# starkware-libs/stark-perpetual

Hardware: AMD Instinct MI355X
Metric: pedersen_hashes_per_sec (higher is better)
Workload: dtype u32x9; 1 GPU; 2^16-leaf Pedersen Merkle rebuild per GPU (BASELINE.json configs[1]), 63 rebuilds in lockstep; tree_height=16, leaves_per_gpu=65536, calls_per_region=28, streams=2, window_bits=26, combine=none

## Files before the change

### stark-perpetual_amd/csrc/curve.hpp

```cpp
#pragma once
#include "fp29.hpp"

namespace sp {

struct aff {
  fe x, y;
};
struct xyzz {
  fe X, Y, ZZ, ZZZ;
};
struct jac {
  fe X, Y, Z;
};

SP_HD xyzz xyzz_from_aff(const aff& p) {
  xyzz r;
  r.X = p.x;
  r.Y = p.y;
  r.ZZ = FE_ONE_M;
  r.ZZZ = FE_ONE_M;
  return r;
}

template <bool SCAN = false>
SP_HD xyzz xyzz_madd(const xyzz& a, const aff& q) {
  if constexpr (SCAN && SP_FE_SCAN) {
    fe t[3];
    fe_scan(t, scan_mul{q.x, a.ZZ}, scan_mul{q.y, a.ZZZ});
    const fe P = fe_sub(t[0], a.X), R = fe_sub(t[1], a.Y);
    const fe P2 = fe_dbl(P), R2 = fe_dbl(R);
    fe_scan(t, scan_sqr{P, P2}, scan_sqr{R, R2});
    const fe PP = t[0], RR = t[1];
    fe_scan(t, scan_mul{P, PP}, scan_mul{a.X, PP});
    const fe PPP = t[0], Q = t[1];
    xyzz r;
    r.X = fe_carry(fe_sub(fe_sub(RR, PPP), fe_dbl(Q)));
    const fe D = fe_sub(Q, r.X), nY = fe_neg_pinned(a.Y);
    fe_scan(t, scan_mul2{R, D, nY, PPP}, scan_mul{a.ZZ, PP}, scan_mul{a.ZZZ, PPP});
    r.Y = t[0];
    r.ZZ = t[1];
    r.ZZZ = t[2];
    return r;
  }
  const fe U2 = fe_mul_t<SCAN>(q.x, a.ZZ);
  const fe S2 = fe_mul_t<SCAN>(q.y, a.ZZZ);
  const fe P = fe_sub(U2, a.X);
  const fe R = fe_sub(S2, a.Y);
  const fe PP = fe_sqr_t<SCAN>(P);
  const fe PPP = fe_mul_t<SCAN>(P, PP);
  const fe Q = fe_mul_t<SCAN>(a.X, PP);
  xyzz r;
  r.X = fe_carry(fe_sub(fe_sub(fe_sqr_t<SCAN>(R), PPP), fe_dbl(Q)));
  r.Y = fe_mul_sub_mul_t<SCAN>(R, fe_sub(Q, r.X), a.Y, PPP);
  r.ZZ = fe_mul_t<SCAN>(a.ZZ, PP);
  r.ZZZ = fe_mul_t<SCAN>(a.ZZZ, PPP);
  return r;
}

template <bool SCAN = false>
SP_HD void xyzz_madd_x_only(const xyzz& a, const aff& q, fe& X3, fe& ZZ3) {
  if constexpr (SCAN && SP_FE_SCAN) {
    fe t[3];
    fe_scan(t, scan_mul{q.x, a.ZZ}, scan_mul{q.y, a.ZZZ});
    const fe P = fe_sub(t[0], a.X), R = fe_sub(t[1], a.Y);
    const fe P2 = fe_dbl(P), R2 = fe_dbl(R);
    fe_scan(t, scan_sqr{P, P2}, scan_sqr{R, R2});
    const fe PP = t[0], RR = t[1];
    fe_scan(t, scan_mul{P, PP}, scan_mul{a.X, PP}, scan_mul{a.ZZ, PP});
    X3 = fe_carry(fe_sub(fe_sub(RR, t[0]), fe_dbl(t[1])));
    ZZ3 = t[2];
    return;
  }
  const fe U2 = fe_mul_t<SCAN>(q.x, a.ZZ);
  const fe S2 = fe_mul_t<SCAN>(q.y, a.ZZZ);
  const fe P = fe_sub(U2, a.X);
  const fe R = fe_sub(S2, a.Y);
  const fe PP = fe_sqr_t<SCAN>(P);
  const fe PPP = fe_mul_t<SCAN>(P, PP);
  const fe Q = fe_mul_t<SCAN>(a.X, PP);
  X3 = fe_carry(fe_sub(fe_sub(fe_sqr_t<SCAN>(R), PPP), fe_dbl(Q)));
  ZZ3 = fe_mul_t<SCAN>(a.ZZ, PP);
}

template <bool SCAN = false>
SP_HD xyzz xyzz_mmadd(const aff& a, const aff& b) {
  if constexpr (SCAN && SP_FE_SCAN) {
    const fe P = fe_sub(b.x, a.x), R = fe_carry(fe_sub(b.y, a.y));
    const fe P2 = fe_dbl(P), R2 = fe_dbl(R);
    fe t[2];
    fe_scan(t, scan_sqr{P, P2}, scan_sqr{R, R2});
    const fe PP = t[0], RR = t[1];
    fe_scan(t, scan_mul{P, PP}, scan_mul{a.x, PP});
    const fe PPP = t[0], Q = t[1];
    xyzz r;
    r.X = fe_carry(fe_sub(fe_sub(RR, PPP), fe_dbl(Q)));
    r.Y = fe_mul_sub_mul_scan(R, fe_sub(Q, r.X), a.y, PPP);
    r.ZZ = PP;
    r.ZZZ = PPP;
    return r;
  }
  const fe P = fe_sub(b.x, a.x);
  const fe R = fe_carry(fe_sub(b.y, a.y));
  const fe PP = fe_sqr_t<SCAN>(P);
  const fe PPP = fe_mul_t<SCAN>(P, PP);
  const fe Q = fe_mul_t<SCAN>(a.x, PP);
  xyzz r;
  r.X = fe_carry(fe_sub(fe_sub(fe_sqr_t<SCAN>(R), PPP), fe_dbl(Q)));
  r.Y = fe_mul_sub_mul_t<SCAN>(R, fe_sub(Q, r.X), a.y, PPP);
  r.ZZ = PP;
  r.ZZZ = PPP;
  return r;
}

template <bool SCAN = false>
SP_HD xyzz xyzz_add(const xyzz& a, const xyzz& b) {
  const fe U1 = fe_mul_t<SCAN>(a.X, b.ZZ);
  const fe U2 = fe_mul_t<SCAN>(b.X, a.ZZ);
  const fe S1 = fe_mul_t<SCAN>(a.Y, b.ZZZ);
  const fe S2 = fe_mul_t<SCAN>(b.Y, a.ZZZ);
  const fe P = fe_sub(U2, U1);
  const fe R = fe_sub(S2, S1);
  const fe PP = fe_sqr_t<SCAN>(P);
  const fe PPP = fe_mul_t<SCAN>(P, PP);
  const fe Q = fe_mul_t<SCAN>(U1, PP);
  xyzz r;
  r.X = fe_carry(fe_sub(fe_sub(fe_sqr_t<SCAN>(R), PPP), fe_dbl(Q)));
  r.Y = fe_mul_sub_mul_t<SCAN>(R, fe_sub(Q, r.X), S1, PPP);
  r.ZZ = fe_mul_t<SCAN>(fe_mul_t<SCAN>(a.ZZ, b.ZZ), PP);
  r.ZZZ = fe_mul_t<SCAN>(fe_mul_t<SCAN>(a.ZZZ, b.ZZZ), PPP);
  return r;
}

template <bool SCAN = false>
SP_HD void xyzz_add_x_only(const xyzz& a, const xyzz& b, fe& X3, fe& ZZ3) {
  const fe U1 = fe_mul_t<SCAN>(a.X, b.ZZ);
  const fe U2 = fe_mul_t<SCAN>(b.X, a.ZZ);
  const fe S1 = fe_mul_t<SCAN>(a.Y, b.ZZZ);
  const fe S2 = fe_mul_t<SCAN>(b.Y, a.ZZZ);
  const fe P = fe_sub(U2, U1);
  const fe R = fe_sub(S2, S1);
  const fe PP = fe_sqr_t<SCAN>(P);
  const fe PPP = fe_mul_t<SCAN>(P, PP);
  const fe Q = fe_mul_t<SCAN>(U1, PP);
  X3 = fe_carry(fe_sub(fe_sub(fe_sqr_t<SCAN>(R), PPP), fe_dbl(Q)));
  ZZ3 = fe_mul_t<SCAN>(fe_mul_t<SCAN>(a.ZZ, b.ZZ), PP);
}

SP_HD jac jac_dbl(const jac& p, const fe& a_coef) {
  const fe XX = fe_sqr(p.X);
  const fe YY = fe_sqr(p.Y);
  const fe YYYY = fe_sqr(YY);
  const fe ZZ = fe_sqr(p.Z);
  const fe t0 = fe_carry(fe_add(p.X, YY));
  const fe halfS = fe_carry(fe_sub(fe_sub(fe_sqr(t0), XX), YYYY));
  const fe S = fe_carry(fe_dbl(halfS));
  const fe XX3 = fe_carry(fe_add(fe_dbl(XX), XX));
  const fe M = fe_carry(fe_add(XX3, fe_mul(a_coef, fe_sqr(ZZ))));
  jac r;
  r.X = fe_carry(fe_sub(fe_sqr(M), fe_dbl(S)));
  const fe y4 = fe_carry(fe_dbl(fe_dbl(YYYY)));
  r.Y = fe_carry(fe_sub(fe_mul(M, fe_sub(S, r.X)), fe_dbl(y4)));
  const fe t1 = fe_carry(fe_add(p.Y, p.Z));
  r.Z = fe_carry(fe_sub(fe_sub(fe_sqr(t1), YY), ZZ));
  return r;
}

struct mjac {
  fe X, Y, Z, W;
};
SP_HD mjac mjac_from(const jac& p, const fe& a_coef) {
  mjac m;
  m.X = p.X; m.Y = p.Y; m.Z = p.Z;
  m.W = fe_mul(a_coef, fe_sqr(fe_sqr(p.Z)));
  return m;
}
SP_HD void mjac_dbl(mjac& p, bool need_w) {
  const fe XX = fe_sqr(p.X);
  const fe YY = fe_sqr(p.Y);
  const fe YYYY = fe_sqr(YY);
  const fe S = fe_carry(fe_dbl(fe_carry(fe_dbl(fe_mul(p.X, YY)))));
  const fe U = fe_carry(fe_dbl(fe_carry(fe_dbl(fe_carry(fe_dbl(YYYY))))));
  const fe M = fe_carry(fe_add(fe_carry(fe_add(fe_dbl(XX), XX)), p.W));
  const fe X3 = fe_carry(fe_sub(fe_sqr(M), fe_dbl(S)));
  const fe Y3 = fe_carry(fe_sub(fe_mul(M, fe_carry(fe_sub(S, X3))), U));
  const fe Z3 = fe_carry(fe_dbl(fe_mul(p.Y, p.Z)));
  if (need_w) p.W = fe_carry(fe_dbl(fe_mul(U, p.W)));
  p.X = X3;
  p.Y = Y3;
  p.Z = Z3;
}

SP_HD jac jac_madd(const jac& p, const aff& q) {
  const fe Z1Z1 = fe_sqr(p.Z);
  const fe U2 = fe_mul(q.x, Z1Z1);
  const fe S2 = fe_mul(fe_mul(q.y, p.Z), Z1Z1);
  const fe H = fe_sub(U2, p.X);
  const fe HH = fe_sqr(H);
  const fe I = fe_dbl(fe_carry(fe_dbl(HH)));
  const fe J = fe_mul(H, I);
  const fe rr = fe_carry(fe_dbl(fe_sub(S2, p.Y)));
  const fe V = fe_mul(p.X, I);
  jac r;
  r.X = fe_carry(fe_sub(fe_sub(fe_sqr(rr), J), fe_dbl(V)));
  r.Y = fe_mul_sub_mul(rr, fe_sub(V, r.X), fe_carry(fe_dbl(p.Y)), J);
  const fe t = fe_carry(fe_add(p.Z, H));
  r.Z = fe_carry(fe_sub(fe_sub(fe_sqr(t), Z1Z1), HH));
  return r;
}

SP_HD jac jac_add(const jac& p, const jac& q) {
  const fe Z1Z1 = fe_sqr(p.Z);
  const fe Z2Z2 = fe_sqr(q.Z);
  const fe U1 = fe_mul(p.X, Z2Z2);
  const fe U2 = fe_mul(q.X, Z1Z1);
  const fe S1 = fe_mul(fe_mul(p.Y, q.Z), Z2Z2);
  const fe S2 = fe_mul(fe_mul(q.Y, p.Z), Z1Z1);
  const fe H = fe_sub(U2, U1);
  const fe I = fe_dbl(fe_carry(fe_dbl(fe_sqr(H))));
  const fe J = fe_mul(H, I);
  const fe rr = fe_carry(fe_dbl(fe_sub(S2, S1)));
  const fe V = fe_mul(U1, I);
  jac r;
  r.X = fe_carry(fe_sub(fe_sub(fe_sqr(rr), J), fe_dbl(V)));
  r.Y = fe_mul_sub_mul(rr, fe_sub(V, r.X), fe_carry(fe_dbl(S1)), J);
  const fe t = fe_carry(fe_add(p.Z, q.Z));
  r.Z = fe_mul(fe_carry(fe_sub(fe_sub(fe_sqr(t), Z1Z1), Z2Z2)), H);
  return r;
}

}
```

### stark-perpetual_amd/csrc/fp29.hpp

```cpp
#pragma once
#include <stdint.h>
#include <utility>

#if defined(__HIPCC__)
#include <hip/hip_runtime.h>
#define SP_HD __host__ __device__ __forceinline__
#else
#define SP_HD inline
#endif

#if defined(SP_CHECK_BOUNDS) && !defined(__HIPCC__)
#include <stdio.h>
#include <stdlib.h>
#define SP_CHK32(expr64)                                                        \
  do {                                                                          \
    long long v__ = (long long)(expr64);                                        \
    if (v__ > 2147483647LL || v__ < -2147483648LL) {                            \
      fprintf(stderr, "limb overflow at %s:%d\n", __FILE__, __LINE__);          \
      abort();                                                                  \
    }                                                                           \
  } while (0)
#define SP_CHK64(expr128)                                                       \
  do {                                                                          \
    __int128 v__ = (expr128);                                                   \
// ... 87 lines not shown
#pragma unroll
  for (int i = 0; i < NL; ++i) r.l[i] = -a.l[i];
  return r;
}
SP_HD fe fe_dbl(const fe& a) {
  fe r;
#pragma unroll
  for (int i = 0; i < NL; ++i) { SP_CHK32((int64_t)a.l[i] * 2); r.l[i] = a.l[i] * 2; }
  return r;
}

SP_HD fe fe_carry(const fe& a) {
  fe r;
  int32_t c = 0;
#pragma unroll
  for (int i = 0; i < 8; ++i) {
    SP_CHK32((int64_t)a.l[i] + c);
    int32_t v = a.l[i] + c;
    r.l[i] = (int32_t)((uint32_t)v & LMASK);
    c = v >> LB;
  }
  r.l[8] = a.l[8] + c;
  return r;
}

SP_HD fe fe_weak_reduce(const fe& a) {
  const int32_t q = a.l[8] >> 19;
  fe r = a;
  r.l[0] -= q;
  r.l[6] -= q * P6;
  r.l[8] -= q * P8;
  return fe_carry(r);
}

SP_HD fe fe_half(const fe& a_in) {
  fe a = fe_carry(a_in);
  const int32_t odd = a.l[0] & 1;
  a.l[0] += odd;
  a.l[6] += odd * P6;
  a.l[8] += odd * P8;
  a = fe_carry(a);
  fe r;
#pragma unroll
  for (int i = 0; i < 8; ++i) r.l[i] = (int32_t)(((uint32_t)a.l[i] >> 1) | (((uint32_t)a.l[i + 1] & 1u) << (LB - 1)));
  r.l[8] = a.l[8] >> 1;
  return r;
}

struct cols {
  int64_t c[17];
};

SP_HD void cols_zero(cols& t) {
#pragma unroll
  for (int i = 0; i < 17; ++i) t.c[i] = 0;
}
SP_HD void cols_mac(cols& t, const fe& a, const fe& b) {
#pragma unroll
  for (int i = 0; i < NL; ++i)
#pragma unroll
    for (int j = 0; j < NL; ++j) {
      SP_CHK64((__int128)t.c[i + j] + (__int128)a.l[i] * b.l[j]);
      t.c[i + j] += (int64_t)a.l[i] * (int64_t)b.l[j];
    }
}
SP_HD void cols_msub(cols& t, const fe& a, const fe& b) {
#pragma unroll
  for (int i = 0; i < NL; ++i)
#pragma unroll
    for (int j = 0; j < NL; ++j) {
      SP_CHK64((__int128)t.c[i + j] - (__int128)a.l[i] * b.l[j]);
      t.c[i + j] -= (int64_t)a.l[i] * (int64_t)b.l[j];
    }
}
SP_HD void cols_sqr(cols& t, const fe& a) {
#pragma unroll
  for (int i = 0; i < NL; ++i) {
    SP_CHK64((__int128)t.c[2 * i] + (__int128)a.l[i] * a.l[i]);
    t.c[2 * i] += (int64_t)a.l[i] * (int64_t)a.l[i];
    SP_CHK32((int64_t)a.l[i] * 2);
    const int32_t d = a.l[i] * 2;
#pragma unroll
    for (int j = i + 1; j < NL; ++j) {
      SP_CHK64((__int128)t.c[i + j] + (__int128)d * a.l[j]);
      t.c[i + j] += (int64_t)d * (int64_t)a.l[j];
    }
  }
}

SP_HD fe fe_reduce(cols& t) {
  int32_t np6 = -P6, np8 = -P8;
#if defined(__HIP_DEVICE_COMPILE__)
  asm volatile("" : "+s"(np6), "+s"(np8));
#endif
#pragma unroll
  for (int i = 0; i < NL; ++i) {
    const int32_t q = (int32_t)((uint32_t)t.c[i] & LMASK);
    t.c[i + 1] += t.c[i] >> LB;
    SP_CHK64((__int128)t.c[i + 6] - (__int128)q * P6);
    t.c[i + 6] += (int64_t)q * (int64_t)np6;
    SP_CHK64((__int128)t.c[i + 8] - ((__int128)q << 19));
    t.c[i + 8] += (int64_t)q * (int64_t)np8;
  }
  fe r;
  int64_t carry = 0;
#pragma unroll
  for (int k = 0; k < 8; ++k) {
    const int64_t v = t.c[9 + k] + carry;
    r.l[k] = (int32_t)((uint32_t)v & LMASK);
    carry = v >> LB;
  }
  SP_CHK32(carry);
  r.l[8] = (int32_t)carry;
  fe_pin(r);
  return r;
}

SP_HD fe fe_mul(const fe& a, const fe& b) {
  cols t;
  cols_zero(t);
  cols_mac(t, a, b);
  return fe_reduce(t);
}
SP_HD fe fe_sqr(const fe& a) {
  cols t;
  cols_zero(t);
  cols_sqr(t, a);
  return fe_reduce(t);
}
SP_HD fe fe_mul_sub_mul(const fe& a, const fe& b, const fe& c, const fe& d) {
  cols t;
  cols_zero(t);
  cols_mac(t, a, b);
  cols_msub(t, c, d);
  return fe_reduce(t);
}
SP_HD fe fe_mul_add_mul(const fe& a, const fe& b, const fe& c, const fe& d) {
  cols t;
  cols_zero(t);
  cols_mac(t, a, b);
  cols_mac(t, c, d);
  return fe_reduce(t);
}

SP_HD fe fe_mul3_add(const fe& a, const fe& b, const fe& c, const fe& d, const fe& e, const fe& f) {
  cols t;
  cols_zero(t);
  cols_mac(t, a, b);
  cols_mac(t, c, d);
  cols_mac(t, e, f);
  return fe_reduce(t);
}

SP_HD void scan_pin(int64_t& acc) {
#if defined(__HIP_DEVICE_COMPILE__)
  asm("" : "+v"(acc));
#else
  (void)acc;
#endif
}
SP_HD void scan_mac(int64_t& acc, int32_t a, int32_t b) {
  SP_CHK64((__int128)acc + (__int128)a * b);
  acc += (int64_t)a * (int64_t)b;
  scan_pin(acc);
}
SP_HD fe fe_neg_pinned(const fe& a) {
  fe r = fe_neg(a);
  fe_pin(r);
  return r;
}
struct scan_mul {
  static constexpr int STEPS = NL;
  const fe &a, &b;
  SP_HD void step(int c, int i, int64_t& acc) const {
    const int j = c - i;
    if (j >= 0 && j < NL) scan_mac(acc, a.l[i], b.l[j]);
  }
};
struct scan_sqr {
  static constexpr int STEPS = NL;
  const fe &a, &d;
  SP_HD void step(int c, int i, int64_t& acc) const {
    const int j = c - i;
    if (j > i && j < NL) scan_mac(acc, d.l[i], a.l[j]);
    if (j == i) scan_mac(acc, a.l[i], a.l[i]);
  }
};
struct scan_mul2 {
  static constexpr int STEPS = 2 * NL;
  const fe &a, &b, &c, &d;
  SP_HD void step(int k, int i, int64_t& acc) const {
    const int j = k - (i % NL);
    if (j >= 0 && j < NL) scan_mac(acc, i < NL ? a.l[i] : c.l[i - NL], i < NL ? b.l[j] : d.l[j]);
  }
};
struct scan_mul3 {
  static constexpr int STEPS = 3 * NL;
  const fe &a, &b, &c, &d, &e, &f;
  SP_HD void step(int k, int i, int64_t& acc) const {
    const int j = k - (i % NL);
    if (j >= 0 && j < NL)
      scan_mac(acc, i < NL ? a.l[i] : i < 2 * NL ? c.l[i - NL] : e.l[i - 2 * NL], i < NL ? b.l[j] : i < 2 * NL ? d.l[j] : f.l[j]);
  }
};
template <int N>
struct scan_state {
  int64_t acc[N];
  int32_t q[N][NL];
  int32_t np6, np8;
};
constexpr int scan_max(int a) { return a; }
template <class... T>
constexpr int scan_max(int a, T... rest) { return a > scan_max(rest...) ? a : scan_max(rest...); }
template <int COL, int I, int N, class... C>
SP_HD void scan_round(scan_state<N>& s, const C&... chains) {
  int k = 0;
  ((I < C::STEPS ? chains.step(COL, I, s.acc[k]) : (void)0, ++k), ...);
}
template <int COL, int N, class... C, int... I>
SP_HD void scan_column(scan_state<N>& s, fe* r, std::integer_sequence<int, I...>, const C&... chains) {
  (scan_round<COL, I>(s, chains...), ...);
  if constexpr (COL >= 6 && COL - 6 < NL) {
#pragma unroll
    for (int k = 0; k < N; ++k) scan_mac(s.acc[k], s.q[k][COL - 6], s.np6);
  }
  if constexpr (COL >= 8) {
#pragma unroll
    for (int k = 0; k < N; ++k) scan_mac(s.acc[k], s.q[k][COL - 8], s.np8);
  }
#pragma unroll
  for (int k = 0; k < N; ++k) {
    const int32_t lo = (int32_t)((uint32_t)s.acc[k] & LMASK);
    if constexpr (COL < NL) s.q[k][COL] = lo; else r[k].l[COL - NL] = lo;
    s.acc[k] >>= LB;
  }
}
template <int N, class... C, int... COL>
SP_HD void scan_columns(scan_state<N>& s, fe* r, std::integer_sequence<int, COL...>, const C&... chains) {
  (scan_column<COL>(s, r, std::make_integer_sequence<int, scan_max(C::STEPS...)>(), chains...), ...);
}
template <class... C>
SP_HD void fe_scan(fe* r, const C&... chains) {
  constexpr int N = sizeof...(C);
  scan_state<N> s;
  s.np6 = -P6;
  s.np8 = -P8;
#if defined(__HIP_DEVICE_COMPILE__)
  asm volatile("" : "+s"(s.np6), "+s"(s.np8));
#endif
#pragma unroll
  for (int k = 0; k < N; ++k) s.acc[k] = 0;
  scan_columns(s, r, std::make_integer_sequence<int, 17>(), chains...);
#pragma unroll
  for (int k = 0; k < N; ++k) {
    SP_CHK32(s.acc[k]);
    r[k].l[8] = (int32_t)s.acc[k];
    fe_pin(r[k]);
  }
}
SP_HD fe fe_mul_scan(const fe& a, const fe& b) {
  fe r;
  fe_scan(&r, scan_mul{a, b});
  return r;
}
SP_HD fe fe_sqr_scan(const fe& a) {
  const fe d = fe_dbl(a);
  fe r;
  fe_scan(&r, scan_sqr{a, d});
  return r;
}
SP_HD fe fe_mul_sub_mul_scan(const fe& a, const fe& b, const fe& c, const fe& d) {
  const fe nc = fe_neg_pinned(c);
  fe r;
  fe_scan(&r, scan_mul2{a, b, nc, d});
  return r;
}
SP_HD fe fe_mul_add_mul_scan(const fe& a, const fe& b, const fe& c, const fe& d) {
  fe r;
  fe_scan(&r, scan_mul2{a, b, c, d});
  return r;
}
SP_HD fe fe_mul3_add_scan(const fe& a, const fe& b, const fe& c, const fe& d, const fe& e, const fe& f) {
  fe r;
  fe_scan(&r, scan_mul3{a, b, c, d, e, f});
  return r;
}

#ifndef SP_FE_SCAN
#define SP_FE_SCAN 1
#endif
template <bool SCAN>
SP_HD fe fe_mul_t(const fe& a, const fe& b) {
  if constexpr (SCAN && SP_FE_SCAN) return fe_mul_scan(a, b);
  else return fe_mul(a, b);
}
template <bool SCAN>
SP_HD fe fe_sqr_t(const fe& a) {
  if constexpr (SCAN && SP_FE_SCAN) return fe_sqr_scan(a);
  else return fe_sqr(a);
}
template <bool SCAN>
SP_HD fe fe_mul_sub_mul_t(const fe& a, const fe& b, const fe& c, const fe& d) {
  if constexpr (SCAN && SP_FE_SCAN) return fe_mul_sub_mul_scan(a, b, c, d);
  else return fe_mul_sub_mul(a, b, c, d);
}

SP_HD bool fe_geq_p_canon_limbs(const fe& a) {
  const bool gt8 = a.l[8] > P8, eq8 = a.l[8] == P8;
  const bool gt6 = a.l[6] > P6, eq6 = a.l[6] == P6;
  const bool low = (a.l[5] | a.l[4] | a.l[3] | a.l[2] | a.l[1]) != 0 || a.l[0] >= 1;
  return gt8 | (eq8 & ((a.l[7] != 0) | gt6 | (eq6 & low)));
}
SP_HD fe fe_canon(const fe& a_in) {
  fe a;
  {
    const int32_t q = a_in.l[8] >> 19;
    a = a_in;
    a.l[0] -= q;
    a.l[6] -= q * P6;
    a.l[8] -= q * P8;
    a = fe_carry(a);
  }
  const int32_t neg = a.l[8] >> 31;
  a.l[0] += neg & 1;
  a.l[6] += neg & P6;
  a.l[8] += neg & P8;
  a = fe_carry(a);
  const int32_t ge = fe_geq_p_canon_limbs(a) ? -1 : 0;
  a.l[0] -= ge & 1;
  a.l[6] -= ge & P6;
  a.l[8] -= ge & P8;
  return fe_carry(a);
}

SP_HD fe fe_to_mont(const fe& a) { return fe_mul(a, FE_R2); }
SP_HD fe fe_from_mont(const fe& a) {
  cols t;
  cols_zero(t);
#pragma unroll
  for (int i = 0; i < NL; ++i) t.c[i] = a.l[i];
  return fe_canon(fe_reduce(t));
}
SP_HD bool fe_is_zero(const fe& a) {
  fe c = fe_from_mont(a);
  int32_t acc = 0;
#pragma unroll
  for (int i = 0; i < NL; ++i) acc |= c.l[i];
  return acc == 0;
}
SP_HD bool fe_eq(const fe& a, const fe& b) { return fe_is_zero(fe_carry(fe_sub(a, b))); }

SP_HD fe fe_sqr_n(fe a, int n) {
  for (int i = 0; i < n; ++i) a = fe_sqr(a);
  return a;
}
SP_HD fe fe_pow_2p59_plus16(const fe& a) {
  fe t = fe_sqr_n(a, 55);
  t = fe_mul(t, a);
  return fe_sqr_n(t, 4);
}
SP_HD fe fe_inv_fermat(const fe& a) {
  fe a2 = fe_sqr(a);
  fe a3 = fe_mul(a2, a);
  fe a7 = fe_mul(fe_sqr(a3), a);
  fe a63 = fe_mul(fe_sqr_n(a7, 3), a7);
  fe r = fe_pow_2p59_plus16(a);
  for (int i = 0; i < 32; ++i) {
    r = fe_sqr_n(r, 6);
    r = fe_mul(r, a63);
  }
  return r;
}
struct trans2x2 {
  int32_t u, v, q, r;
};

SP_HD int32_t divsteps_29(int32_t zeta, uint32_t f0, uint32_t g0, trans2x2& t) {
  uint32_t u = 1, v = 0, q = 0, r = 1;
  uint32_t f = f0, g = g0;
  for (int i = 0; i < LB; ++i) {
    uint32_t c1 = (uint32_t)(zeta >> 31);
    const uint32_t c2 = 0u - (g & 1u);
    const uint32_t x = (f ^ c1) - c1;
    const uint32_t y = (u ^ c1) - c1;
    const uint32_t z = (v ^ c1) - c1;
    g += x & c2;
    q += y & c2;
    r += z & c2;
    c1 &= c2;
    zeta = (int32_t)((uint32_t)zeta ^ c1) - 1;
    f += g & c1;
    u += q & c1;
// ... 528 lines not shown
```

### stark-perpetual_amd/csrc/pedersen.hip

```cpp
#include <algorithm>
#include <cstdlib>
#include <cstring>
#include <map>
#include <vector>

#include "context.hpp"
#include "quad.hpp"

#ifndef SP_ACC_WAVES
#define SP_ACC_WAVES 1
#endif

namespace sp {

struct raw_aff {
  u256 x, y;
};
__device__ __forceinline__ raw_aff ld_raw(const aff_packed* e) {
  const uint4* q = reinterpret_cast<const uint4*>(e);
  const uint4 a = q[0], b = q[1], c = q[2], d = q[3];
  raw_aff r;
  r.x.w[0] = a.x; r.x.w[1] = a.y; r.x.w[2] = a.z; r.x.w[3] = a.w;
  r.x.w[4] = b.x; r.x.w[5] = b.y; r.x.w[6] = b.z; r.x.w[7] = b.w;
  r.y.w[0] = c.x; r.y.w[1] = c.y; r.y.w[2] = c.z; r.y.w[3] = c.w;
  r.y.w[4] = d.x; r.y.w[5] = d.y; r.y.w[6] = d.z; r.y.w[7] = d.w;
  return r;
}
__device__ __forceinline__ aff unpack_raw(const raw_aff& t) {
  aff r;
  r.x = fe_unpack(t.x);
  r.y = fe_unpack(t.y);
  return r;
}

struct bits512 {
  uint32_t w[16];
};
__device__ __forceinline__ bits512 concat_xy(const u256& x, const u256& y) {
  bits512 s;
#pragma unroll
  for (int i = 0; i < 7; ++i) s.w[i] = x.w[i];
  s.w[7] = x.w[7] | (y.w[0] << 28);
#pragma unroll
  for (int i = 0; i < 7; ++i) s.w[8 + i] = (y.w[i] >> 4) | (y.w[i + 1] << 28);
  s.w[15] = y.w[7] >> 4;
  return s;
}
__device__ __forceinline__ uint32_t pop_bits(bits512& s, int width) {
  const uint32_t v = s.w[0] & ((1u << width) - 1u);
  bits512 n;
#pragma unroll
  for (int i = 0; i < 15; ++i) n.w[i] = __builtin_amdgcn_alignbit(s.w[i + 1], s.w[i], (uint32_t)width);
  n.w[15] = s.w[15] >> width;
  s = n;
  return v;
}
struct window_ref {
  const aff_packed* entry;
  bool negative;
};
__device__ __forceinline__ window_ref window_entry(const aff_packed* __restrict__ ped, int g, uint32_t raw,
                                                    int w0, int log2e) {
  window_ref r;
  if (g == 0) {
    r.entry = ped + raw;
    r.negative = false;
  } else {
    const uint32_t mask = (1u << log2e) - 1u;
    r.negative = (raw >> log2e) == 0;
    const uint32_t idx = r.negative ? (~raw & mask) : (raw & mask);
    r.entry = ped + ((size_t)1 << w0) + ((size_t)(g - 1) << log2e) + idx;
  }
  return r;
}
__device__ __forceinline__ int window_width(int g, int w0, int log2e) { return g == 0 ? w0 : log2e + 1; }
__device__ __forceinline__ int window_start(int g, int w0, int log2e) {
  return g == 0 ? 0 : w0 + (g - 1) * (log2e + 1);
}
__device__ __forceinline__ aff signed_aff(const raw_aff& t, bool negative) {
  aff q = unpack_raw(t);
  if (negative) q.y = fe_neg(q.y);
  return q;
}

__device__ __forceinline__ void store_limbs(int32_t* base, size_t n, size_t e, const fe& v) {
#pragma unroll
  for (int k = 0; k < NL; ++k) base[(size_t)k * n + e] = v.l[k];
}
__device__ __forceinline__ fe load_limbs(const int32_t* base, size_t n, size_t e) {
  fe v;
#pragma unroll
  for (int k = 0; k < NL; ++k) v.l[k] = base[(size_t)k * n + e];
  return v;
}

__device__ __forceinline__ void operand_pointers(const uint64_t* x, const uint64_t* y, size_t xstride,
                                                 size_t ystride, const int2* __restrict__ src, size_t e,
                                                 const uint64_t*& fx, const uint64_t*& fy) {
  if (src == nullptr) {
    fx = x + 4 * e * xstride;
    fy = y + 4 * e * ystride;
  } else {
    const int2 s = src[e];
    fx = s.x >= 0 ? x + 4 * (size_t)s.x : y;
    fy = s.y >= 0 ? x + 4 * (size_t)s.y : y;
  }
}

#ifndef SP_SCAN_BULK
#define SP_SCAN_BULK true
#endif
#ifndef SP_SCAN_SPLIT
#define SP_SCAN_SPLIT false
#endif

__device__ __forceinline__ void
bulk_accumulate(const uint64_t* __restrict__ x, const uint64_t* __restrict__ y, size_t xstride,
                size_t ystride, size_t n, const aff_packed* __restrict__ ped, int w0, int log2e,
                int nwin, int32_t* __restrict__ sX, int32_t* __restrict__ sZZ,
                uint8_t* __restrict__ status, unsigned* __restrict__ flag,
                const int2* __restrict__ src, size_t plane, size_t e) {
  if (e >= n) return;
  const uint64_t *fx, *fy;
  operand_pointers(x, y, xstride, ystride, src, e, fx, fy);
  u256 sx = ld_u256(fx);
  u256 sy = ld_u256(fy);
  uint8_t st = SP_HASH_OK;
  if (!u256_lt(sx, U256_P) || !u256_lt(sy, U256_P)) {
    st = SP_HASH_OUT_OF_RANGE;
#pragma unroll
    for (int i = 0; i < 8; ++i) { sx.w[i] = 0; sy.w[i] = 0; }
  }
  bits512 str = concat_xy(sx, sy);
  auto next_window = [&](int g) {
    return window_entry(ped, g, pop_bits(str, window_width(g, w0, log2e)), w0, log2e);
  };
  const raw_aff e0 = ld_raw(next_window(0).entry);
  window_ref r1 = next_window(1 < nwin ? 1 : 0);
  raw_aff n1 = ld_raw(r1.entry);
  bool neg1 = r1.negative, neg2 = false;
  raw_aff n2 = n1;
  if (nwin > 2) {
    const window_ref r2 = next_window(2);
    n2 = ld_raw(r2.entry);
    neg2 = r2.negative;
  }
  xyzz acc;
  int first = 1;
  if (nwin > 2) {
    const aff q1 = signed_aff(n1, neg1);
    n1 = n2;
    neg1 = neg2;
    if (3 < nwin) {
      const window_ref r = next_window(3);
      n2 = ld_raw(r.entry);
      neg2 = r.negative;
    }
    acc = xyzz_mmadd<SP_SCAN_BULK>(unpack_raw(e0), q1);
    first = 2;
  } else {
    acc = xyzz_from_aff(unpack_raw(e0));
  }
  for (int i = first; i + 1 < nwin; ++i) {
    const aff q = signed_aff(n1, neg1);
    n1 = n2;
    neg1 = neg2;
    if (i + 2 < nwin) {
      const window_ref r = next_window(i + 2);
      n2 = ld_raw(r.entry);
      neg2 = r.negative;
    }
    acc = xyzz_madd<SP_SCAN_BULK>(acc, q);
  }
  if (nwin > 1) {
    fe X3, ZZ3;
    xyzz_madd_x_only<SP_SCAN_BULK>(acc, signed_aff(n1, neg1), X3, ZZ3);
    store_limbs(sX, plane, e, X3);
    store_limbs(sZZ, plane, e, ZZ3);
  } else {
    store_limbs(sX, plane, e, acc.X);
    store_limbs(sZZ, plane, e, acc.ZZ);
  }
  if (st != SP_HASH_OK) {
    if (status) status[e] = st;
    if (flag) atomicOr(flag, (unsigned)st);
  } else if (status) {
    status[e] = SP_HASH_OK;
  }
}

__global__ void __launch_bounds__(256, SP_ACC_WAVES)
ped_accumulate_kernel(const uint64_t* __restrict__ x, const uint64_t* __restrict__ y, size_t xstride,
                      size_t ystride, size_t n, const aff_packed* __restrict__ ped, int w0, int log2e,
                      int nwin, int32_t* __restrict__ sX, int32_t* __restrict__ sZZ,
                      uint8_t* __restrict__ status, unsigned* __restrict__ flag,
                      const int2* __restrict__ src, size_t plane) {
  bulk_accumulate(x, y, xstride, ystride, n, ped, w0, log2e, nwin, sX, sZZ, status, flag, src, plane,
                  (size_t)blockIdx.x * blockDim.x + threadIdx.x);
}

__device__ __forceinline__ fe shfl_xor_fe(const fe& v, int mask) {
  fe r;
#pragma unroll
  for (int i = 0; i < NL; ++i) r.l[i] = __shfl_xor(v.l[i], mask, 64);
  return r;
}
__device__ __forceinline__ uint32_t field_from_memory(const uint64_t* felt, int bit, int width) {
  const uint32_t* w = reinterpret_cast<const uint32_t*>(felt);
  const int wi = bit >> 5, sh = bit & 31;
  uint64_t two = (uint64_t)w[wi];
  if (wi + 1 < 8) two |= (uint64_t)w[wi + 1] << 32;
  return (uint32_t)(two >> sh) & ((1u << width) - 1u);
}
__device__ __forceinline__ uint32_t window_from_memory(const uint64_t* fx, const uint64_t* fy, int start,
                                                       int width) {
  if (start + width <= 252) return field_from_memory(fx, start, width);
  if (start >= 252) return field_from_memory(fy, start - 252, width);
  const int lo_n = 252 - start;
  return field_from_memory(fx, start, lo_n) | (field_from_memory(fy, 0, width - lo_n) << lo_n);
}

template <int LOG_L>
__device__ __forceinline__ xyzz split_accumulate(const uint64_t* fx, const uint64_t* fy, int sub,
                                                 const aff_packed* __restrict__ ped, int w0, int log2e,
                                                 int nwin) {
  constexpr int L = 1 << LOG_L;
  const int cnt_lo = nwin / L, extra = nwin % L;
  const int cnt = cnt_lo + (sub < extra ? 1 : 0);
  const int g0 = sub * cnt_lo + (sub < extra ? sub : extra);
  auto entry = [&](int g) {
    return window_entry(ped, g, window_from_memory(fx, fy, window_start(g, w0, log2e), window_width(g, w0, log2e)),
                        w0, log2e);
  };
  const window_ref r0 = entry(g0);
  const aff q0 = signed_aff(ld_raw(r0.entry), r0.negative);
  window_ref rn = entry(g0 + 1);
  raw_aff nxt = ld_raw(rn.entry);
  xyzz acc;
  {
    const aff q1 = signed_aff(nxt, rn.negative);
    if (cnt > 2) {
      rn = entry(g0 + 2);
      nxt = ld_raw(rn.entry);
    }
    acc = xyzz_mmadd<SP_SCAN_SPLIT>(q0, q1);
  }
  for (int j = 2; j < cnt; ++j) {
    const aff q = signed_aff(nxt, rn.negative);
    if (j + 1 < cnt) {
      rn = entry(g0 + j + 1);
      nxt = ld_raw(rn.entry);
    }
    acc = xyzz_madd<SP_SCAN_SPLIT>(acc, q);
  }
#pragma unroll 1
  for (int r = 0; r + 1 < LOG_L; ++r) {
    xyzz o;
    o.X = shfl_xor_fe(acc.X, 1 << r);
    o.Y = shfl_xor_fe(acc.Y, 1 << r);
    o.ZZ = shfl_xor_fe(acc.ZZ, 1 << r);
    o.ZZZ = shfl_xor_fe(acc.ZZZ, 1 << r);
    acc = xyzz_add<SP_SCAN_SPLIT>(acc, o);
  }
  if constexpr (LOG_L > 0) {
    constexpr int r = LOG_L - 1;
    xyzz o;
// ... 237 lines not shown
                 unsigned* __restrict__ flag, uint64_t* __restrict__ out, int dup) {
  constexpr int QUADS = 1 << LOG_Q, LANES = 4 * QUADS;
  __shared__ uint64_t slot[256 / LANES][4];
  const size_t gt = (size_t)blockIdx.x * blockDim.x + threadIdx.x;
  const size_t e_raw = gt / ((size_t)LANES << dup);
  const int g = (int)(gt % LANES), grp = (int)(threadIdx.x / LANES);
  const bool active = e_raw < n;
  const size_t e = active ? e_raw : n - 1;
  const uint64_t* h = first + 4 * e;
  const uint64_t* w = words + 4 * e;
  for (int j = 0; j < steps; ++j, w += 4 * word_stride) {
    const uint64_t* fx = h_right ? w : h;
    const uint64_t* fy = h_right ? h : w;
    bool unhashable;
    const u256 xa = quad_hash<LOG_Q, false>(fx, fy, 0, nullptr, 0, 0, ped, w0, log2e, nwin_plan, g, &unhashable);
    uint8_t st = unhashable ? SP_HASH_UNHASHABLE : SP_HASH_OK;
    if (g == 0 && (!u256_lt(ld_u256(w), U256_P) || (j == 0 && !u256_lt(ld_u256(h), U256_P)))) st = SP_HASH_OUT_OF_RANGE;
    __syncthreads();
    if (g == 0) {
      uint32_t* sl = reinterpret_cast<uint32_t*>(slot[grp]);
#pragma unroll
      for (int k = 0; k < 8; ++k) sl[k] = xa.w[k];
      if (active) {
        if (j == steps - 1) st_u256(out + 4 * e, xa);
        if (st != SP_HASH_OK && flag) atomicOr(flag, (unsigned)st);
      }
    }
    __syncthreads();
    h = slot[grp];
  }
}

template <int LOG_Q>
__global__ void __launch_bounds__(256)
ped_chain_ragged_kernel(const uint64_t* __restrict__ elems, const uint32_t* __restrict__ off, size_t n,
                        const aff_packed* __restrict__ ped, int w0, int log2e, int nwin_plan,
                        unsigned* __restrict__ flag, uint8_t* __restrict__ status, uint64_t* __restrict__ out, int dup) {
  constexpr int QUADS = 1 << LOG_Q, LANES = 4 * QUADS;
  __shared__ uint64_t slot[256 / LANES][4];
  __shared__ int block_steps;
  const size_t gt = (size_t)blockIdx.x * blockDim.x + threadIdx.x;
  const size_t e_raw = gt / ((size_t)LANES << dup);
  const int g = (int)(gt % LANES), grp = (int)(threadIdx.x / LANES);
  const bool active = e_raw < n;
  const size_t e = active ? e_raw : n - 1;
  const bool writer = active && g == 0 && ((gt / LANES) & (((size_t)1 << dup) - 1)) == 0;
  const uint32_t o0 = off[e];
  const int steps = (int)(off[e + 1] - o0) - 1;
  if (threadIdx.x == 0) block_steps = 0;
  __syncthreads();
  if (g == 0 && steps > 0) atomicMax(&block_steps, steps);
  __syncthreads();
  const int bound = block_steps;
  const uint64_t* e0 = elems + 4 * (size_t)o0;
  uint8_t st = SP_HASH_OK;
  if (steps == 0 && writer) {
    const u256 v = ld_u256(e0);
    if (!u256_lt(v, U256_P)) st = SP_HASH_OUT_OF_RANGE;
    st_u256(out + 4 * e, v);
    if (status) status[e] = st;
    if (st != SP_HASH_OK && flag) atomicOr(flag, (unsigned)st);
  }
  const uint64_t* h = e0;
  const uint64_t* w = e0 + 4;
  for (int j = 0; j < bound; ++j, w += 4) {
    const bool live = j < steps;
    const uint64_t* fx = live ? h : e0;
    const uint64_t* fy = live ? w : e0;
    bool unhashable;
    const u256 xa = quad_hash<LOG_Q, false>(fx, fy, 0, nullptr, 0, 0, ped, w0, log2e, nwin_plan, g, &unhashable);
    if (live && g == 0) {
      if (!u256_lt(ld_u256(w), U256_P) || (j == 0 && !u256_lt(ld_u256(h), U256_P))) st |= SP_HASH_OUT_OF_RANGE;
      else if (unhashable) st |= SP_HASH_UNHASHABLE;
    }
    __syncthreads();
    if (live && g == 0) {
      uint32_t* sl = reinterpret_cast<uint32_t*>(slot[grp]);
#pragma unroll
      for (int k = 0; k < 8; ++k) sl[k] = xa.w[k];
      if (j == steps - 1 && writer) {
        st_u256(out + 4 * e, xa);
        if (status) status[e] = st;
        if (st != SP_HASH_OK && flag) atomicOr(flag, (unsigned)st);
      }
    }
    __syncthreads();
    h = slot[grp];
  }
}

__global__ void __launch_bounds__(256)
ped_chain_ragged_scatter_kernel(const uint64_t* __restrict__ work, const uint64_t* __restrict__ elems,
                                const uint32_t* __restrict__ off, const uint32_t* __restrict__ perm,
                                const uint32_t* __restrict__ step_off, const uint8_t* __restrict__ step_status, size_t n,
                                unsigned* __restrict__ flag, uint8_t* __restrict__ status, uint64_t* __restrict__ out) {
  const size_t k = (size_t)blockIdx.x * blockDim.x + threadIdx.x;
  if (k >= n) return;
  const uint32_t c = perm[k];
  const uint32_t o0 = off[c], len = off[c + 1] - o0;
  uint8_t st = SP_HASH_OK;
  u256 v;
  if (len == 1) {
    v = ld_u256(elems + 4 * (size_t)o0);
    if (!u256_lt(v, U256_P)) st = SP_HASH_OUT_OF_RANGE;
    if (st != SP_HASH_OK && flag) atomicOr(flag, (unsigned)st);
  } else {
    v = ld_u256(work + 4 * k);
    for (uint32_t j = 1; j < len; ++j) st |= step_status[(size_t)step_off[j] + k];
  }
  st_u256(out + 4 * (size_t)c, v);
  if (status) status[c] = st;
}

__global__ void __launch_bounds__(256)
ped_top_kernel(uint64_t* __restrict__ cur, size_t n_in, int n_levels, const aff_packed* __restrict__ ped, int w0, int log2e,
               int nwin_plan, unsigned* __restrict__ flag) {
  constexpr int LANES = 32, GROUPS = 256 / LANES;
  __shared__ uint64_t slot[2][GROUPS][4];
  const int g = (int)(threadIdx.x % LANES), grp = (int)(threadIdx.x / LANES);
  const size_t b = blockIdx.x;
  const int chunk = 1 << n_levels;
  uint64_t* out = cur + 4 * n_in;
  size_t n_out = n_in >> 1;
  int share = 4 - n_levels;
  for (int t = 0; t < n_levels; ++t, ++share) {
    const int cnt = chunk >> (t + 1);
    const int i = grp >> share;
    const bool writer = g == 0 && (grp & ((1 << share) - 1)) == 0;
    const uint64_t *fx, *fy;
    if (t == 0) {
      fx = cur + 4 * ((size_t)chunk * b + 2 * (size_t)i);
      fy = fx + 4;
    } else {
      fx = slot[(t - 1) & 1][2 * i];
      fy = slot[(t - 1) & 1][2 * i + 1];
    }
    bool unhashable;
    const u256 xa = quad_hash<3, false>(fx, fy, 0, nullptr, 0, 0, ped, w0, log2e, nwin_plan, g, &unhashable);
    uint8_t st = unhashable ? SP_HASH_UNHASHABLE : SP_HASH_OK;
    if (t == 0 && writer && (!u256_lt(ld_u256(fx), U256_P) || !u256_lt(ld_u256(fy), U256_P))) st = SP_HASH_OUT_OF_RANGE;
    if (writer) {
      uint32_t* sl = reinterpret_cast<uint32_t*>(slot[t & 1][i]);
#pragma unroll
      for (int w = 0; w < 8; ++w) sl[w] = xa.w[w];
      st_u256(out + 4 * ((size_t)cnt * b + (size_t)i), xa);
      if (st != SP_HASH_OK && flag) atomicOr(flag, (unsigned)st);
    }
    __syncthreads();
    out += 4 * n_out;
    n_out >>= 1;
  }
}

__global__ void __launch_bounds__(256)
ped_finish_kernel(const int32_t* __restrict__ sX, int32_t* __restrict__ sZZ, int32_t* __restrict__ sPre,
                  size_t n, size_t T, uint64_t* __restrict__ out, size_t ostride,
                  uint8_t* __restrict__ status, unsigned* __restrict__ flag) {
  const size_t t = (size_t)blockIdx.x * blockDim.x + threadIdx.x;
  if (t >= T) return;
  const size_t cnt = t < n ? (n - t + T - 1) / T : 0;
  fe run = FE_ONE_M;
  if (cnt > 0) {
    fe znext = load_limbs(sZZ, n, t);
#pragma unroll 1
    for (size_t j = 0; j < cnt; ++j) {
      const size_t e = t + j * T;
      const fe z = znext;
      if (j + 1 < cnt) znext = load_limbs(sZZ, n, e + T);
      store_limbs(sPre, n, e, run);
      run = fe_mul(run, z);
    }
  }
  if (fe_is_zero(run)) {
    run = FE_ONE_M;
#pragma unroll 1
    for (size_t e = t; e < n; e += T) {
      fe z = load_limbs(sZZ, n, e);
      if (fe_is_zero(z)) {
        z = FE_ONE_M;
        store_limbs(sZZ, n, e, z);
        if (status) status[e] = SP_HASH_UNHASHABLE;
        if (flag) atomicOr(flag, (unsigned)SP_HASH_UNHASHABLE);
      }
      store_limbs(sPre, n, e, run);
      run = fe_mul(run, z);
    }
  }
  size_t e = cnt > 0 ? t + (cnt - 1) * T : 0;
  fe zn = run, pn = run, xn = run;
  if (cnt > 0) {
    zn = load_limbs(sZZ, n, e);
    pn = load_limbs(sPre, n, e);
    xn = load_limbs(sX, n, e);
  }
  fe inv = fe_inv_shared_quad<2, true>(run, (int)(threadIdx.x & 3));
#pragma unroll 1
  for (size_t j = cnt; j-- > 0;) {
    const fe z = zn, pre = pn, xv = xn;
    const size_t cur = t + j * T;
    if (j > 0) {
      zn = load_limbs(sZZ, n, cur - T);
      pn = load_limbs(sPre, n, cur - T);
      xn = load_limbs(sX, n, cur - T);
    }
    const fe zinv = fe_mul(inv, pre);
    inv = fe_mul(inv, z);
    const fe xa = fe_mul(xv, zinv);
    st_u256(out + 4 * cur * ostride, fe_pack(fe_canon(xa)));
  }
}

template <bool Z_IN_LDS>
__global__ void __launch_bounds__(256)
ped_finish_lds_kernel(const int32_t* __restrict__ sX, int32_t* __restrict__ sZZ, size_t n, size_t T,
                      uint64_t* __restrict__ out, size_t ostride, uint8_t* __restrict__ status,
                      unsigned* __restrict__ flag, int kmax) {
  extern __shared__ int32_t fin_lds[];
  int32_t* lpre = fin_lds;
  int32_t* lz = fin_lds + (size_t)kmax * NL * 256;
  auto lds_put = [&](int32_t* base, size_t j, const fe& v) {
#pragma unroll
    for (int k = 0; k < NL; ++k) base[((j * NL + k) << 8) + threadIdx.x] = v.l[k];
  };
  auto lds_get = [&](const int32_t* base, size_t j) {
    fe v;
#pragma unroll
    for (int k = 0; k < NL; ++k) v.l[k] = base[((j * NL + k) << 8) + threadIdx.x];
    return v;
  };
  const size_t t = (size_t)blockIdx.x * blockDim.x + threadIdx.x;
  if (t >= T) return;
  const size_t cnt = t < n ? (n - t + T - 1) / T : 0;
  fe run = FE_ONE_M;
  if (cnt > 0) {
    fe znext = load_limbs(sZZ, n, t);
#pragma unroll 1
    for (size_t j = 0; j < cnt; ++j) {
      const fe z = znext;
      if (j + 1 < cnt) znext = load_limbs(sZZ, n, t + (j + 1) * T);
      lds_put(lpre, j, run);
      if (Z_IN_LDS) lds_put(lz, j, z);
      run = fe_mul(run, z);
    }
  }
  if (fe_is_zero(run)) {
    run = FE_ONE_M;
    size_t j = 0;
#pragma unroll 1
    for (size_t e = t; e < n; e += T, ++j) {
      fe z = load_limbs(sZZ, n, e);
      if (fe_is_zero(z)) {
        z = FE_ONE_M;
        store_limbs(sZZ, n, e, z);
        if (status) status[e] = SP_HASH_UNHASHABLE;
        if (flag) atomicOr(flag, (unsigned)SP_HASH_UNHASHABLE);
      }
      lds_put(lpre, j, run);
      if (Z_IN_LDS) lds_put(lz, j, z);
      run = fe_mul(run, z);
    }
  }
  size_t e = cnt > 0 ? t + (cnt - 1) * T : 0;
  fe zn = run, xn = run;
  if (cnt > 0) {
    if (!Z_IN_LDS) zn = load_limbs(sZZ, n, e);
    xn = load_limbs(sX, n, e);
  }
  fe inv = fe_inv_shared_quad<2, true>(run, (int)(threadIdx.x & 3));
#pragma unroll 1
  for (size_t j = cnt; j-- > 0;) {
    const fe z = Z_IN_LDS ? lds_get(lz, j) : zn, xv = xn;
    const fe pre = lds_get(lpre, j);
    const size_t cur = t + j * T;
    if (j > 0) {
      if (!Z_IN_LDS) zn = load_limbs(sZZ, n, cur - T);
      xn = load_limbs(sX, n, cur - T);
    }
    const fe zinv = fe_mul(inv, pre);
    inv = fe_mul(inv, z);
    const fe xa = fe_mul(xv, zinv);
    st_u256(out + 4 * cur * ostride, fe_pack(fe_canon(xa)));
  }
}

__global__ void __launch_bounds__(128)
ped_point_kernel(const uint64_t* __restrict__ x, const uint64_t* __restrict__ y, size_t n,
                 const aff_packed* __restrict__ ped, int w0, int log2e, int nwin,
                 uint64_t* __restrict__ ox, uint64_t* __restrict__ oy, uint8_t* __restrict__ status) {
  size_t e = (size_t)blockIdx.x * blockDim.x + threadIdx.x;
  if (e >= n) e = n - 1;
  u256 sx = ld_u256(x + 4 * e);
  u256 sy = ld_u256(y + 4 * e);
  if (!u256_lt(sx, U256_P) || !u256_lt(sy, U256_P)) {
    status[e] = SP_HASH_OUT_OF_RANGE;
    return;
  }
  bits512 str = concat_xy(sx, sy);
  xyzz acc = xyzz_from_aff(ld_aff(ped + pop_bits(str, w0)));
  for (int g = 1; g < nwin; ++g) {
    const window_ref r = window_entry(ped, g, pop_bits(str, log2e + 1), w0, log2e);
    acc = xyzz_madd(acc, signed_aff(ld_raw(r.entry), r.negative));
  }
  if (fe_is_zero(acc.ZZ)) {
    status[e] = SP_HASH_UNHASHABLE;
    return;
  }
  const fe izzz = fe_inv(acc.ZZZ);
  st_u256(ox + 4 * e, fe_pack(fe_from_mont(fe_mul(acc.X, fe_sqr(fe_mul(acc.ZZ, izzz))))));
  st_u256(oy + 4 * e, fe_pack(fe_from_mont(fe_mul(acc.Y, izzz))));
  status[e] = SP_HASH_OK;
}

__global__ void __launch_bounds__(64)
ped_partial_kernel(const uint64_t* __restrict__ felts, int count, const aff_packed* __restrict__ ped, int w0, int log2e,
                   int nwin, int cx, int cy, aff_packed* __restrict__ out) {
  int t = (int)(blockIdx.x * blockDim.x + threadIdx.x);
  if (t >= 2 * count) t = 2 * count - 1;
  const int side = t & 1;
  const uint64_t* f = felts + 4 * (size_t)(t >> 1);
  const int g0 = side == 0 ? 0 : nwin - cy, g1 = side == 0 ? cx : nwin;
  auto entry = [&](int w) {
    const window_ref r =
        window_entry(ped, w, window_from_memory(f, f, window_start(w, w0, log2e), window_width(w, w0, log2e)), w0, log2e);
    return signed_aff(ld_raw(r.entry), r.negative);
  };
  aff_packed res;
  if (g1 - g0 == 1) {
    const aff a = entry(g0);
    res.x = fe_pack(fe_canon(a.x));
    res.y = fe_pack(fe_canon(a.y));
  } else {
    xyzz acc = xyzz_mmadd(entry(g0), entry(g0 + 1));
    for (int g = g0 + 2; g < g1; ++g) acc = xyzz_madd(acc, entry(g));
    const fe izzz = fe_inv(acc.ZZZ);
    const fe izz = fe_sqr(fe_mul(acc.ZZ, izzz));
    res.x = fe_pack(fe_canon(fe_mul(acc.X, izz)));
    res.y = fe_pack(fe_canon(fe_mul(acc.Y, izzz)));
  }
  uint4* q = reinterpret_cast<uint4*>(out + t);
  q[0] = make_uint4(res.x.w[0], res.x.w[1], res.x.w[2], res.x.w[3]);
  q[1] = make_uint4(res.x.w[4], res.x.w[5], res.x.w[6], res.x.w[7]);
  q[2] = make_uint4(res.y.w[0], res.y.w[1], res.y.w[2], res.y.w[3]);
  q[3] = make_uint4(res.y.w[4], res.y.w[5], res.y.w[6], res.y.w[7]);
}

struct KernelProfile {
  bool enabled = false;
  std::vector<hipEvent_t> ev;
  std::vector<size_t> units;
  size_t used = 0;
};
static KernelProfile g_prof;
static bool g_split_enabled = getenv("STARKPERP_NO_SPLIT") == nullptr;
static bool g_fuse_enabled = getenv("STARKPERP_NO_FUSE") == nullptr;
static bool g_quad_enabled = getenv("STARKPERP_NO_QUAD") == nullptr;
static bool g_quad2_enabled = getenv("STARKPERP_NO_QUAD2") == nullptr;
static bool g_level_split = getenv("STARKPERP_NO_LEVEL_SPLIT") == nullptr;
static bool g_quad_no_dup = getenv("STARKPERP_QUAD_NO_DUP") != nullptr;
static bool g_sparse_enabled = getenv("STARKPERP_NO_SPARSE_LEVELS") == nullptr;
static size_t g_quad_max = getenv("STARKPERP_QUAD_MAX") ? (size_t)atoll(getenv("STARKPERP_QUAD_MAX")) : 2048;
struct Scratch {
  int32_t *X, *ZZ, *Pre;
  unsigned* flag;
};
static std::map<StreamKey, DeviceBuffer> g_stream_scratch;
int get_scratch_public(size_t n, Scratch& s, hipStream_t st);
static int get_scratch(size_t n, Scratch& s, hipStream_t st) { return get_scratch_public(n, s, st); }
static int get_scratch_tail(size_t n, size_t tail_bytes, Scratch& s, char** tail, hipStream_t st) {
  DeviceBuffer& buf = g_stream_scratch[stream_key(st)];
  const size_t plane = ((9 * n * sizeof(int32_t)) + 255) & ~(size_t)255;
  SP_HIP(buf.reserve(3 * plane + 256 + tail_bytes));
  char* b = (char*)buf.ptr;
  s.X = (int32_t*)b;
  s.ZZ = (int32_t*)(b + plane);
  s.Pre = (int32_t*)(b + 2 * plane);
  s.flag = (unsigned*)(b + 3 * plane);
  if (tail) *tail = b + 3 * plane + 256;
  return SP_OK;
}
int get_scratch_public(size_t n, Scratch& s, hipStream_t st) { return get_scratch_tail(n, 0, s, nullptr, st); }

static size_t g_finish_lanes = getenv("STARKPERP_FINISH_LANES") ? (size_t)atoll(getenv("STARKPERP_FINISH_LANES")) : 65536;
static size_t parse_split_lanes() {
  const char* e = getenv("STARKPERP_SPLIT_LANES");
  long long v = e ? atoll(e) : 65536;
  if (v < 256) v = 256;
  if (v > (1ll << 24)) v = 1ll << 24;
  return ((size_t)v + 255) & ~(size_t)255;
}
static size_t g_split_lanes = parse_split_lanes();
static bool g_finish_lds = getenv("STARKPERP_NO_FINISH_LDS") == nullptr;
static int finish_lds_ready() {
  static std::map<int, int> done;
  int dev = -1;
  if (hipGetDevice(&dev) != hipSuccess) return SP_ERR_HIP;
  auto it = done.find(dev);
  if (it != done.end()) return it->second;
  const int want = 16 * NL * 256 * (int)sizeof(int32_t);
  hipError_t e = hipFuncSetAttribute(reinterpret_cast<const void*>(ped_finish_lds_kernel<true>),
                                     hipFuncAttributeMaxDynamicSharedMemorySize, want);
  if (e == hipSuccess)
    e = hipFuncSetAttribute(reinterpret_cast<const void*>(ped_finish_lds_kernel<false>),
                            hipFuncAttributeMaxDynamicSharedMemorySize, want);
  if (e != hipSuccess) (void)hipGetLastError();
  return done[dev] = (e == hipSuccess ? SP_OK : SP_ERR_HIP);
}
static size_t finish_threads(size_t n) {
  size_t K = (n + g_finish_lanes - 1) / g_finish_lanes;
  if (K < 1) K = 1;
  if (K > 32) K = 32;
  return ((n + K - 1) / K + 3) & ~(size_t)3;
}

void release_ragged_stage();
void release_pedersen_state() {
  for (auto& kv : g_stream_scratch) kv.second.release();
  g_stream_scratch.clear();
  release_ragged_stage();
  for (hipEvent_t e : g_prof.ev) (void)hipEventDestroy(e);
  g_prof.ev.clear();
  g_prof.units.clear();
// ... 703 lines not shown
```

Baseline: 1.039 billion hashes/s.

## Interleave field multiplies via scan chains in xyzz_add and finish kernels

Adds scan-fused (interleaved multi-chain) versions of xyzz_add and xyzz_add_x_only, reorders the round interleaving inside fe_scan, and inserts configurable sched_barrier fences. The finish kernels' backward pass is rewritten so the three per-element multiplies run as one interleaved scan, overlapping successive iterations. SP_SCAN_SPLIT is also enabled by default. The goal is more instruction-level parallelism in the 29-bit-limb field arithmetic, at the cost of higher register pressure and scheduler constraints that may hurt occupancy.

```diff
diff --git a/stark-perpetual_amd/csrc/curve.hpp b/stark-perpetual_amd/csrc/curve.hpp
--- a/stark-perpetual_amd/csrc/curve.hpp
+++ b/stark-perpetual_amd/csrc/curve.hpp
@@ -36,9 +36,9 @@
     xyzz r;
     r.X = fe_carry(fe_sub(fe_sub(RR, PPP), fe_dbl(Q)));
     const fe D = fe_sub(Q, r.X), nY = fe_neg_pinned(a.Y);
-    fe_scan(t, scan_mul2{R, D, nY, PPP}, scan_mul{a.ZZ, PP}, scan_mul{a.ZZZ, PPP});
-    r.Y = t[0];
-    r.ZZ = t[1];
+    fe_scan(t, scan_mul{a.ZZ, PP}, scan_mul2{R, D, nY, PPP}, scan_mul{a.ZZZ, PPP});
+    r.ZZ = t[0];
+    r.Y = t[1];
     r.ZZZ = t[2];
     return r;
   }
@@ -94,7 +94,7 @@
     const fe PPP = t[0], Q = t[1];
     xyzz r;
     r.X = fe_carry(fe_sub(fe_sub(RR, PPP), fe_dbl(Q)));
-    r.Y = fe_mul_sub_mul_scan(R, fe_sub(Q, r.X), a.y, PPP);
+    r.Y = fe_mul_sub_mul(R, fe_sub(Q, r.X), a.y, PPP);
     r.ZZ = PP;
     r.ZZZ = PPP;
     return r;
@@ -114,6 +114,26 @@
 
 template <bool SCAN = false>
 SP_HD xyzz xyzz_add(const xyzz& a, const xyzz& b) {
+  if constexpr (SCAN && SP_FE_SCAN) {
+    fe t[3];
+    fe_scan(t, scan_mul{a.X, b.ZZ}, scan_mul{b.X, a.ZZ}, scan_mul{a.Y, b.ZZZ});
+    const fe U1 = t[0], S1 = t[2], P = fe_sub(t[1], t[0]);
+    fe_scan(t, scan_mul{b.Y, a.ZZZ}, scan_mul{a.ZZ, b.ZZ}, scan_mul{a.ZZZ, b.ZZZ});
+    const fe R = fe_sub(t[0], S1), Zab = t[1], Zzab = t[2];
+    const fe P2 = fe_dbl(P), R2 = fe_dbl(R);
+    fe_scan(t, scan_sqr{P, P2}, scan_sqr{R, R2});
+    const fe PP = t[0], RR = t[1];
+    fe_scan(t, scan_mul{P, PP}, scan_mul{U1, PP});
+    const fe PPP = t[0], Q = t[1];
+    xyzz r;
+    r.X = fe_carry(fe_sub(fe_sub(RR, PPP), fe_dbl(Q)));
+    const fe D = fe_sub(Q, r.X), nS1 = fe_neg_pinned(S1);
+    fe_scan(t, scan_mul{Zab, PP}, scan_mul2{R, D, nS1, PPP}, scan_mul{Zzab, PPP});
+    r.ZZ = t[0];
+    r.Y = t[1];
+    r.ZZZ = t[2];
+    return r;
+  }
   const fe U1 = fe_mul_t<SCAN>(a.X, b.ZZ);
   const fe U2 = fe_mul_t<SCAN>(b.X, a.ZZ);
   const fe S1 = fe_mul_t<SCAN>(a.Y, b.ZZZ);
@@ -133,6 +153,20 @@
 
 template <bool SCAN = false>
 SP_HD void xyzz_add_x_only(const xyzz& a, const xyzz& b, fe& X3, fe& ZZ3) {
+  if constexpr (SCAN && SP_FE_SCAN) {
+    fe t[3];
+    fe_scan(t, scan_mul{a.X, b.ZZ}, scan_mul{b.X, a.ZZ}, scan_mul{a.Y, b.ZZZ});
+    const fe U1 = t[0], S1 = t[2], P = fe_sub(t[1], t[0]);
+    fe_scan(t, scan_mul{b.Y, a.ZZZ}, scan_mul{a.ZZ, b.ZZ});
+    const fe R = fe_sub(t[0], S1), Zab = t[1];
+    const fe P2 = fe_dbl(P), R2 = fe_dbl(R);
+    fe_scan(t, scan_sqr{P, P2}, scan_sqr{R, R2});
+    const fe PP = t[0], RR = t[1];
+    fe_scan(t, scan_mul{P, PP}, scan_mul{U1, PP}, scan_mul{Zab, PP});
+    X3 = fe_carry(fe_sub(fe_sub(RR, t[0]), fe_dbl(t[1])));
+    ZZ3 = t[2];
+    return;
+  }
   const fe U1 = fe_mul_t<SCAN>(a.X, b.ZZ);
   const fe U2 = fe_mul_t<SCAN>(b.X, a.ZZ);
   const fe S1 = fe_mul_t<SCAN>(a.Y, b.ZZZ);
diff --git a/stark-perpetual_amd/csrc/fp29.hpp b/stark-perpetual_amd/csrc/fp29.hpp
--- a/stark-perpetual_amd/csrc/fp29.hpp
+++ b/stark-perpetual_amd/csrc/fp29.hpp
@@ -263,17 +263,27 @@
   return fe_reduce(t);
 }
 
+#ifndef SP_SCAN_ORDER
+#define SP_SCAN_ORDER 2
+#endif
 SP_HD void scan_pin(int64_t& acc) {
 #if defined(__HIP_DEVICE_COMPILE__)
   asm("" : "+v"(acc));
 #else
   (void)acc;
+#endif
+}
+template <int LEVEL>
+SP_HD void scan_fence() {
+#if defined(__HIP_DEVICE_COMPILE__)
+  if constexpr (SP_SCAN_ORDER == LEVEL) __builtin_amdgcn_sched_barrier(0);
 #endif
 }
 SP_HD void scan_mac(int64_t& acc, int32_t a, int32_t b) {
   SP_CHK64((__int128)acc + (__int128)a * b);
   acc += (int64_t)a * (int64_t)b;
   scan_pin(acc);
+  scan_fence<2>();
 }
 SP_HD fe fe_neg_pinned(const fe& a) {
   fe r = fe_neg(a);
@@ -327,28 +337,34 @@
 SP_HD void scan_round(scan_state<N>& s, const C&... chains) {
   int k = 0;
   ((I < C::STEPS ? chains.step(COL, I, s.acc[k]) : (void)0, ++k), ...);
-}
-template <int COL, int N, class... C, int... I>
-SP_HD void scan_column(scan_state<N>& s, fe* r, std::integer_sequence<int, I...>, const C&... chains) {
-  (scan_round<COL, I>(s, chains...), ...);
+  scan_fence<1>();
+}
+template <int COL, int M, int N, class... C, int... J>
+SP_HD void scan_column(scan_state<N>& s, fe* r, std::integer_sequence<int, J...>, const C&... chains) {
+  (scan_round<COL, (J % M) * NL + J / M>(s, chains...), ...);
   if constexpr (COL >= 6 && COL - 6 < NL) {
 #pragma unroll
     for (int k = 0; k < N; ++k) scan_mac(s.acc[k], s.q[k][COL - 6], s.np6);
+    scan_fence<1>();
   }
   if constexpr (COL >= 8) {
 #pragma unroll
     for (int k = 0; k < N; ++k) scan_mac(s.acc[k], s.q[k][COL - 8], s.np8);
+    scan_fence<1>();
   }
 #pragma unroll
   for (int k = 0; k < N; ++k) {
     const int32_t lo = (int32_t)((uint32_t)s.acc[k] & LMASK);
     if constexpr (COL < NL) s.q[k][COL] = lo; else r[k].l[COL - NL] = lo;
     s.acc[k] >>= LB;
-  }
+    if constexpr (N > 1) scan_fence<2>();
+  }
+  scan_fence<1>();
 }
 template <int N, class... C, int... COL>
 SP_HD void scan_columns(scan_state<N>& s, fe* r, std::integer_sequence<int, COL...>, const C&... chains) {
-  (scan_column<COL>(s, r, std::make_integer_sequence<int, scan_max(C::STEPS...)>(), chains...), ...);
+  constexpr int M = scan_max(C::STEPS...) / NL;
+  (scan_column<COL, M>(s, r, std::make_integer_sequence<int, NL * M>(), chains...), ...);
 }
 template <class... C>
 SP_HD void fe_scan(fe* r, const C&... chains) {
diff --git a/stark-perpetual_amd/csrc/pedersen.hip b/stark-perpetual_amd/csrc/pedersen.hip
--- a/stark-perpetual_amd/csrc/pedersen.hip
+++ b/stark-perpetual_amd/csrc/pedersen.hip
@@ -111,7 +111,10 @@
 #define SP_SCAN_BULK true
 #endif
 #ifndef SP_SCAN_SPLIT
-#define SP_SCAN_SPLIT false
+#define SP_SCAN_SPLIT true
+#endif
+#ifndef SP_SCAN_FINISH
+#define SP_SCAN_FINISH true
 #endif
 
 __device__ __forceinline__ void
@@ -655,6 +658,27 @@
   }
 }
 
+template <class Fetch, class Emit>
+__device__ __forceinline__ void finish_backward_scan(fe inv, size_t cnt, Fetch fetch, Emit emit) {
+  if (cnt == 0) return;
+  fe z, pre, xv, r[3];
+  fetch(cnt - 1, z, pre, xv);
+  fe_scan(r, scan_mul{inv, pre}, scan_mul{inv, z});
+  fe zinv = r[0];
+  inv = r[1];
+#pragma unroll 1
+  for (size_t j = cnt - 1; j-- > 0;) {
+    fe xn;
+    fetch(j, z, pre, xn);
+    fe_scan(r, scan_mul{inv, pre}, scan_mul{inv, z}, scan_mul{xv, zinv});
+    emit(j + 1, r[2]);
+    zinv = r[0];
+    inv = r[1];
+    xv = xn;
+  }
+  emit(0, fe_mul(xv, zinv));
+}
+
 __global__ void __launch_bounds__(256)
 ped_finish_kernel(const int32_t* __restrict__ sX, int32_t* __restrict__ sZZ, int32_t* __restrict__ sPre,
                   size_t n, size_t T, uint64_t* __restrict__ out, size_t ostride,
@@ -697,6 +721,21 @@
     xn = load_limbs(sX, n, e);
   }
   fe inv = fe_inv_shared_quad<2, true>(run, (int)(threadIdx.x & 3));
+  if constexpr (SP_SCAN_FINISH && SP_FE_SCAN) {
+    finish_backward_scan(
+        inv, cnt,
+        [&](size_t j, fe& z, fe& pre, fe& xv) {
+          z = zn; pre = pn; xv = xn;
+          if (j > 0) {
+            const size_t nx = t + (j - 1) * T;
+            zn = load_limbs(sZZ, n, nx);
+            pn = load_limbs(sPre, n, nx);
+            xn = load_limbs(sX, n, nx);
+          }
+        },
+        [&](size_t j, const fe& xa) { st_u256(out + 4 * (t + j * T) * ostride, fe_pack(fe_canon(xa))); });
+    return;
+  }
 #pragma unroll 1
   for (size_t j = cnt; j-- > 0;) {
     const fe z = zn, pre = pn, xv = xn;
@@ -770,6 +809,22 @@
     xn = load_limbs(sX, n, e);
   }
   fe inv = fe_inv_shared_quad<2, true>(run, (int)(threadIdx.x & 3));
+  if constexpr (SP_SCAN_FINISH && SP_FE_SCAN) {
+    finish_backward_scan(
+        inv, cnt,
+        [&](size_t j, fe& z, fe& pre, fe& xv) {
+          z = Z_IN_LDS ? lds_get(lz, j) : zn;
+          pre = lds_get(lpre, j);
+          xv = xn;
+          if (j > 0) {
+            const size_t nx = t + (j - 1) * T;
+            if (!Z_IN_LDS) zn = load_limbs(sZZ, n, nx);
+            xn = load_limbs(sX, n, nx);
+          }
+        },
+        [&](size_t j, const fe& xa) { st_u256(out + 4 * (t + j * T) * ostride, fe_pack(fe_canon(xa))); });
+    return;
+  }
 #pragma unroll 1
   for (size_t j = cnt; j-- > 0;) {
     const fe z = Z_IN_LDS ? lds_get(lz, j) : zn, xv = xn;
```

Result: no change. 1.044 billion hashes/s, median of 6 (+0.5%).
